# caslabuiowa/OptimalBezierTrajectoryGeneration

Measured on NVIDIA B200. Metric: constraint+Jacobian evals/sec, higher is better.
Workload: dtype f64

## Files before the change

### optimalbeziertrajectorygeneration_b200/csrc/common.cuh

```cuda
#pragma once
#include <cuda_runtime.h>
#include <stdint.h>
#include <stdio.h>
#include <string.h>

#include "bezgpu.h"

struct bez_plan {
    int n, dim, elev, device;
    int L;
    int Lh;
    int LhPad;
    double *d_PQ;
    double *d_T;
    double *d_W;
    double *d_E1;
    double h_W[(BEZ_MAX_DEGREE + 1) * (BEZ_MAX_DEGREE + 1)];
    double h_E1lo[BEZ_MAX_DEGREE + 1];
    double h_E1hi[BEZ_MAX_DEGREE + 1];
};

void bez_set_error(const char *fmt, ...);
int bez_cuda_fail(cudaError_t e, const char *what);

#define BEZ_CUDA(call)                                        \
    do {                                                      \
        cudaError_t e__ = (call);                             \
        if (e__ != cudaSuccess) return bez_cuda_fail(e__, #call); \
    } while (0)

struct BezDeviceGuard {
    int prev = -1;
    bool switched = false;
    cudaError_t err = cudaSuccess;
    explicit BezDeviceGuard(int device) {
        err = cudaGetDevice(&prev);
        if (err == cudaSuccess && prev != device) {
            err = cudaSetDevice(device);
            switched = (err == cudaSuccess);
        }
    }
    ~BezDeviceGuard() {
        if (switched) cudaSetDevice(prev);
    }
    BezDeviceGuard(const BezDeviceGuard &) = delete;
    BezDeviceGuard &operator=(const BezDeviceGuard &) = delete;
};
#define BEZ_ON_DEVICE(device)                                                     \
    BezDeviceGuard bez_guard__(device);                                            \
    if (bez_guard__.err != cudaSuccess) return bez_cuda_fail(bez_guard__.err, "cudaSetDevice")

int bez_kernel_config(const void *func, int threads, size_t shmem, int *sms, int *ctas_per_sm);

#define BEZ_REQUIRE(cond, msg)                 \
    do {                                       \
        if (!(cond)) {                         \
            bez_set_error("%s: %s", __func__, msg); \
            return BEZ_EINVAL;                 \
        }                                      \
    } while (0)

__host__ __device__ inline long long bez_pair_row_offset(long long i, long long N) {
    return i * (2 * N - i - 1) / 2;
}

__device__ inline void bez_pair_decode(long long p, int N, int &i, int &j) {
    const float b = 2.0f * (float)N - 1.0f;
    const float disc = (float)((2.0 * (double)N - 1.0) * (2.0 * (double)N - 1.0) - 8.0 * (double)p);
    int ii = (int)((b - __fsqrt_rn(disc > 0.0f ? disc : 0.0f)) * 0.5f);
    if (ii < 0) ii = 0;
    if (ii > N - 2) ii = N - 2;
    while (ii > 0 && bez_pair_row_offset(ii, N) > p) --ii;
    while (ii < N - 2 && bez_pair_row_offset(ii + 1, N) <= p) ++ii;
    i = ii;
    j = (int)(p - bez_pair_row_offset(ii, N)) + ii + 1;
}
```

### optimalbeziertrajectorygeneration_b200/csrc/plan.cu

```cuda
#include <stdarg.h>
#include <stdlib.h>

#include <mutex>
#include <vector>

#include "common.cuh"

static thread_local char g_err[512] = "";

void bez_set_error(const char *fmt, ...) {
    va_list ap;
    va_start(ap, fmt);
    vsnprintf(g_err, sizeof(g_err), fmt, ap);
    va_end(ap);
}

int bez_cuda_fail(cudaError_t e, const char *what) {
    bez_set_error("CUDA error %d (%s) in %s", (int)e, cudaGetErrorString(e), what);
    return (int)e;
}

extern "C" const char *bez_last_error(void) { return g_err; }

namespace {
struct KernelConfig {
    const void *func;
    int device, threads;
    size_t shmem;
    int sms, per_sm;
};
std::mutex g_cfg_mutex;
std::vector<KernelConfig> g_cfg;
}

int bez_kernel_config(const void *func, int threads, size_t shmem, int *sms, int *ctas_per_sm) {
    int dev = 0;
    BEZ_CUDA(cudaGetDevice(&dev));
    std::lock_guard<std::mutex> lock(g_cfg_mutex);
    for (const KernelConfig &c : g_cfg)
        if (c.func == func && c.device == dev && c.threads == threads && c.shmem == shmem) {
            *sms = c.sms;
            *ctas_per_sm = c.per_sm;
            return BEZ_OK;
        }
    KernelConfig c{func, dev, threads, shmem, 148, 1};
    size_t granted = 48 * 1024;
    for (const KernelConfig &o : g_cfg)
        if (o.func == func && o.device == dev && o.shmem > granted) granted = o.shmem;
    if (shmem > granted)
        BEZ_CUDA(cudaFuncSetAttribute(func, cudaFuncAttributeMaxDynamicSharedMemorySize, (int)shmem));
    BEZ_CUDA(cudaDeviceGetAttribute(&c.sms, cudaDevAttrMultiProcessorCount, dev));
    BEZ_CUDA(cudaOccupancyMaxActiveBlocksPerMultiprocessor(&c.per_sm, func, threads, shmem));
    if (c.per_sm < 1) c.per_sm = 1;
    g_cfg.push_back(c);
    *sms = c.sms;
    *ctas_per_sm = c.per_sm;
    return BEZ_OK;
}
extern "C" int bez_version(void) { return 100; }

extern "C" int bez_plan_create(int n, int dim, int elev, int device,
                               const double *h_prodW, const double *h_elevT,
                               const double *h_elev1, bez_plan **out) {
    BEZ_REQUIRE(out != nullptr, "out is NULL");
    *out = nullptr;
    BEZ_REQUIRE(h_prodW && h_elevT, "tables are NULL");
    BEZ_REQUIRE(dim >= 1 && dim <= 3, "dim must be 1, 2 or 3");
    BEZ_REQUIRE(elev >= 0, "elev must be >= 0");
    if (n < 1 || n > BEZ_MAX_DEGREE) {
        bez_set_error("bez_plan_create: degree %d outside [1, %d]", n, BEZ_MAX_DEGREE);
        return BEZ_EUNSUPPORTED;
    }
    BEZ_REQUIRE(h_elev1 != nullptr, "elev1 table is NULL");
    BEZ_ON_DEVICE(device);

    bez_plan *p = (bez_plan *)calloc(1, sizeof(bez_plan));
    if (!p) {
        bez_set_error("bez_plan_create: out of host memory");
        return BEZ_ENOMEM;
    }
    p->n = n; p->dim = dim; p->elev = elev; p->device = device;
    const int m = 2 * n;
    p->L = m + elev + 1;
    p->Lh = (p->L + 1) / 2;
    p->LhPad = (p->Lh + 31) / 32 * 32;
    const int L = p->L, M = m + elev;

    memcpy(p->h_W, h_prodW, sizeof(double) * (n + 1) * (n + 1));
    for (int i = 0; i <= n; ++i) {
        p->h_E1lo[i] = (i < n) ? h_elev1[i * (n + 1) + i] : 0.0;
        p->h_E1hi[i] = (i > 0) ? h_elev1[(i - 1) * (n + 1) + i] : 0.0;
    }

    std::vector<double> PQ((size_t)(m + 1) * p->LhPad, 0.0);
    for (int i = 0; i < p->Lh; ++i) {
        for (int j = 0; j < n; ++j) {
            double a = h_elevT[(size_t)j * L + i], b = h_elevT[(size_t)(m - j) * L + i];
            PQ[(size_t)j * p->LhPad + i] = (a + b) * 0.5;
            PQ[(size_t)(n + 1 + j) * p->LhPad + i] = (a - b) * 0.5;
        }
        PQ[(size_t)n * p->LhPad + i] = h_elevT[(size_t)n * L + i];
    }
    for (int i = p->Lh; i < p->LhPad; ++i) {
        const int mi = M - i;
        if (mi < 0 || mi >= p->Lh) continue;
        for (int j = 0; j <= n; ++j) PQ[(size_t)j * p->LhPad + i] = PQ[(size_t)j * p->LhPad + mi];
        for (int j = 0; j < n; ++j)
            PQ[(size_t)(n + 1 + j) * p->LhPad + i] = -PQ[(size_t)(n + 1 + j) * p->LhPad + mi];
    }

    cudaError_t e;
#define PLAN_ALLOC_COPY(dst, src, count)                                              \
    e = cudaMalloc((void **)&(dst), sizeof(double) * (count));                        \
    if (e == cudaSuccess)                                                             \
        e = cudaMemcpy((dst), (src), sizeof(double) * (count), cudaMemcpyHostToDevice); \
    if (e != cudaSuccess) { bez_plan_destroy(p); return bez_cuda_fail(e, "plan table upload"); }
    PLAN_ALLOC_COPY(p->d_PQ, PQ.data(), PQ.size());
    PLAN_ALLOC_COPY(p->d_T, h_elevT, (size_t)(m + 1) * L);
    PLAN_ALLOC_COPY(p->d_W, h_prodW, (size_t)(n + 1) * (n + 1));
    PLAN_ALLOC_COPY(p->d_E1, h_elev1, (size_t)n * (n + 1));
#undef PLAN_ALLOC_COPY
    *out = p;
    return BEZ_OK;
}

extern "C" int bez_plan_destroy(bez_plan *p) {
    if (!p) return BEZ_OK;
    cudaFree(p->d_PQ);
    cudaFree(p->d_T);
    cudaFree(p->d_W);
    cudaFree(p->d_E1);
    free(p);
    return BEZ_OK;
}

extern "C" int bez_plan_info(const bez_plan *p, int *n, int *dim, int *elev, int *L) {
    BEZ_REQUIRE(p != nullptr, "plan is NULL");
    if (n) *n = p->n;
    if (dim) *dim = p->dim;
    if (elev) *elev = p->elev;
    if (L) *L = p->L;
    return BEZ_OK;
}
```

### optimalbeziertrajectorygeneration_b200/csrc/sq_elev_ws.cuh

```cuda
#pragma once
#include "sq_elev_stage1.cuh"

namespace bezws {
using namespace bezcore;
using namespace bezmma;

constexpr int kProducers = 4, kConsumers = 8;
constexpr int kWsThreads = 32 * (kProducers + kConsumers);
constexpr int kSlots = 3;
constexpr int kBarsPerGroup = 3 * kSlots;

template <int R> __device__ __forceinline__ void reg_dec() { asm volatile("setmaxnreg.dec.sync.aligned.u32 %0;" :: "n"(R)); }
template <int R> __device__ __forceinline__ void reg_inc() { asm volatile("setmaxnreg.inc.sync.aligned.u32 %0;" :: "n"(R)); }
__device__ __forceinline__ void mbar_arrive(unsigned mbar_s) {
    asm volatile("mbarrier.arrive.shared::cta.b64 _, [%0];" :: "r"(mbar_s) : "memory");
}

template <int N_, int DIM> __host__ __device__ constexpr int slot_doubles() {
    constexpr int S_ = (DIM * (N_ + 1) + 1) / 2 * 2;
    return 32 * S_ > kRowsDoubles ? 32 * S_ : kRowsDoubles;
}

template <int N_, int DIM, int MINMODE, bool STORE>
__global__ void __launch_bounds__(kWsThreads, 1)
sq_elev_ws_kernel(const SqElevArgs A, const ProdWeights<N_> PW, const DiffWeights<N_> DW) {
    constexpr int NP = 4;
    constexpr int S_ = (DIM * (N_ + 1) + 1) / 2 * 2;
    constexpr int kSlotD = slot_doubles<N_, DIM>();
    extern __shared__ __align__(16) double smem[];
    const int lane = threadIdx.x & 31;
    const int warp = __shfl_sync(0xffffffffu, (int)(threadIdx.x >> 5), 0);
    const int group = warp & 3;
    double *slots = smem + (size_t)group * kSlots * kSlotD;
    double *stag0 = smem + (size_t)4 * kSlots * kSlotD;
    const size_t stag_per = STORE ? 16 * (size_t)A.L : 0;
    const unsigned bars_s = (unsigned)__cvta_generic_to_shared(stag0 + kConsumers * stag_per) + 8u * kBarsPerGroup * group;
    auto full_b = [&](int s) { return bars_s + 8u * s; };
    auto empty_b = [&](int s) { return bars_s + 8u * (kSlots + s); };
    auto rows_b = [&](int s) { return bars_s + 8u * (2 * kSlots + s); };
    if (warp < kProducers && lane == 0) {
        for (int s = 0; s < kSlots; ++s) { mbar_init(full_b(s), 32); mbar_init(empty_b(s), 32); mbar_init(rows_b(s), 1); }
        mbar_fence_init();
    }
    __syncthreads();

    const long long total = A.nitems * (long long)A.B;
    const long long nwt = (total + 31) >> 5;
    const long long ngroups = (long long)gridDim.x * 4, gidx = (long long)blockIdx.x * 4 + group;
    const long long t_begin = gidx * nwt / ngroups;
    const int n = (int)((gidx + 1) * nwt / ngroups - t_begin);

    if (warp < kProducers) {
        reg_dec<120>();
        PairCursor cur;
        if (n > 0) {
            const long long f = (t_begin << 5) + lane;
            cur = pair_cursor_at(A, f < total ? f : total - 1);
        }
        for (int k = 0; k < n; ++k) {
            const int s = k % kSlots, use = k / kSlots;
            double *slot = slots + (size_t)s * kSlotD;
            const unsigned slot_s = (unsigned)__cvta_generic_to_shared(slot);
            if (use > 0) mbar_wait(empty_b(s), (unsigned)(use - 1) & 1u);
            {
                const int pb = __shfl_up_sync(0xffffffffu, cur.b, 1), pi = __shfl_up_sync(0xffffffffu, cur.i, 1);
                const int pj = __shfl_up_sync(0xffffffffu, cur.j, 1);
                const bool start = lane == 0 || cur.b != pb || cur.i != pi || cur.j != pj + 1;
                const unsigned runs = __ballot_sync(0xffffffffu, start);
                if (lane == 0) mbar_arrive_expect_tx(rows_b(s), 32u * S_ * 8u);
                __syncwarp();
                if (start) {
                    const unsigned higher = lane == 31 ? 0u : (runs & (0xffffffffu << (lane + 1)));
                    const int end = higher ? __ffs(higher) - 1 : 32;
                    bulk_load(slot_s + (unsigned)lane * (S_ * 8u), A.cpts + ((size_t)cur.b * A.N + cur.j) * S_,
                              (unsigned)(end - lane) * (S_ * 8u), rows_b(s));
                }
            }
            const long long g0 = (t_begin + k) << 5;
            PairCursor nxt = cur;
            if (k + 1 < n) {
                const long long fn = g0 + 32 + lane;
                nxt = fn < total ? pair_cursor_next(A, cur, g0 + lane) : pair_cursor_at(A, total - 1);
            }
            mbar_wait(rows_b(s), (unsigned)use & 1u);
            double sc[2 * N_ + 1];
            stage1_coeffs<N_, DIM, PAIR, true>(A, PW, DW, cur.b, cur.i, cur.j, sc, slot + lane * S_);
            __syncwarp();
            double *row = slot + lane * kRowStride;
#pragma unroll
            for (int j = 0; j < N_; ++j) {
                row[slot_e(j)] = sc[j] + sc[2 * N_ - j];
                row[slot_o(j)] = sc[j] - sc[2 * N_ - j];
            }
            row[slot_e(N_)] = sc[N_];
#pragma unroll
            for (int j = N_ + 1; j < 4 * Geom<N_>::KE; ++j) row[slot_e(j)] = 0.0;
#pragma unroll
            for (int j = N_; j < 4 * Geom<N_>::KO; ++j) row[slot_o(j)] = 0.0;
            mbar_arrive(full_b(s));
            cur = nxt;
        }
    } else {
        reg_inc<192>();
        const int cidx = warp - kProducers, ci = cidx >> 2;
        double *obuf = stag0 + (size_t)cidx * stag_per;
        const unsigned obuf_s = (unsigned)__cvta_generic_to_shared(obuf);
        const bool base_aligned = (reinterpret_cast<uintptr_t>(A.out) & 15u) == 0;
        BFrags<N_, NP> Bf;
        load_bfrags<N_, NP>(Bf, A.PQ, A.L, A.LhPad, lane);
        for (int k = ci; k < n; k += 2) {
            const int s = k % kSlots, use = k / kSlots;
            const long long g0 = (t_begin + k) << 5;
            const int cnt = (int)((total - g0) < 32 ? (total - g0) : 32);
            mbar_wait(full_b(s), (unsigned)use & 1u);
            auto release = [&]() { mbar_arrive(empty_b(s)); };
            mma_tile<N_, NP, MINMODE, STORE, decltype(release)>(slots + (size_t)s * kSlotD, obuf, obuf_s, Bf,
                                                                STORE ? A.out + (size_t)g0 * A.L : nullptr, A.sinks, g0, cnt,
                                                                A.L, A.beta, lane, base_aligned, false, release);
            __syncwarp();
        }
        if (STORE && lane == 0) bulk_wait_all();
    }
}

template <int N_, int DIM> size_t ws_shmem_bytes(int L, bool store) {
    return ((size_t)4 * kSlots * slot_doubles<N_, DIM>() + (store ? (size_t)kConsumers * 16 * L : 0) + 4 * kBarsPerGroup) *
           sizeof(double);
}
template <int N_, int DIM> bool ws_fits(int L, bool store) { return ws_shmem_bytes<N_, DIM>(L, store) <= 232448; }

template <int N_, int DIM, int MINMODE, bool STORE>
int launch_sq_elev_ws(const bez_plan *plan, const SqElevArgs &A, cudaStream_t st) {
    ProdWeights<N_> PW;
    DiffWeights<N_> DW;
    const double scale = A.alpha * (0.5 * (double)DIM);
    for (int i = 0; i <= N_; ++i)
        for (int j = i; j <= N_; ++j) {
            double w = plan->h_W[i * (N_ + 1) + j] * scale;
            PW.w[widx<N_>(i, j)] = (i == j) ? w : 2.0 * w;
        }
    for (int i = 0; i <= N_; ++i) { DW.lo[i] = plan->h_E1lo[i]; DW.hi[i] = plan->h_E1hi[i]; }
    const size_t shmem = ws_shmem_bytes<N_, DIM>(A.L, STORE);
    auto kern = sq_elev_ws_kernel<N_, DIM, MINMODE, STORE>;
    int sms = 148, per_sm = 1;
    if (int rc = bez_kernel_config((const void *)kern, kWsThreads, shmem, &sms, &per_sm)) return rc;
    const long long nwt = (A.nitems * (long long)A.B + 31) / 32;
    long long grid = sms;
    if (grid > (nwt + 7) / 8) grid = (nwt + 7) / 8;
    if (grid == sms && grid > 1 && !(A.flags & kFlagFullGrid)) grid -= 1;
    if (grid < 1) return BEZ_OK;
    kern<<<(unsigned)grid, kWsThreads, shmem, st>>>(A, PW, DW);
    BEZ_CUDA(cudaGetLastError());
    return BEZ_OK;
}

}
```

Baseline: 12190.

## Replace static tile split in warp-specialized kernel with atomic dynamic work claiming

Each producer group now claims chunks of two 32-item tiles from a global atomic counter instead of taking a fixed contiguous range. Producers write the tile index into shared memory for consumers and send sentinel slots to end the loop. The last group to finish resets the counter, and each launch takes its counter pair from a ring on the plan. This is meant to even out load across groups when per-tile cost or group speed varies, at the cost of atomic traffic, a cursor re-seek at every chunk boundary, and a new launch-size limit.

```diff
diff --git a/optimalbeziertrajectorygeneration_b200/csrc/common.cuh b/optimalbeziertrajectorygeneration_b200/csrc/common.cuh
--- a/optimalbeziertrajectorygeneration_b200/csrc/common.cuh
+++ b/optimalbeziertrajectorygeneration_b200/csrc/common.cuh
@@ -18,7 +18,10 @@
     double h_W[(BEZ_MAX_DEGREE + 1) * (BEZ_MAX_DEGREE + 1)];
     double h_E1lo[BEZ_MAX_DEGREE + 1];
     double h_E1hi[BEZ_MAX_DEGREE + 1];
+    unsigned *d_ws_work;
+    mutable unsigned ws_work_next;
 };
+constexpr int kWsWorkRing = 64;
 
 void bez_set_error(const char *fmt, ...);
 int bez_cuda_fail(cudaError_t e, const char *what);
diff --git a/optimalbeziertrajectorygeneration_b200/csrc/plan.cu b/optimalbeziertrajectorygeneration_b200/csrc/plan.cu
--- a/optimalbeziertrajectorygeneration_b200/csrc/plan.cu
+++ b/optimalbeziertrajectorygeneration_b200/csrc/plan.cu
@@ -120,6 +120,10 @@
     PLAN_ALLOC_COPY(p->d_W, h_prodW, (size_t)(n + 1) * (n + 1));
     PLAN_ALLOC_COPY(p->d_E1, h_elev1, (size_t)n * (n + 1));
 #undef PLAN_ALLOC_COPY
+    e = cudaMalloc((void **)&p->d_ws_work, sizeof(unsigned) * 2 * kWsWorkRing);
+    if (e == cudaSuccess) e = cudaMemset(p->d_ws_work, 0, sizeof(unsigned) * 2 * kWsWorkRing);
+    if (e == cudaSuccess) e = cudaDeviceSynchronize();
+    if (e != cudaSuccess) { bez_plan_destroy(p); return bez_cuda_fail(e, "plan work counters"); }
     *out = p;
     return BEZ_OK;
 }
@@ -130,6 +134,7 @@
     cudaFree(p->d_T);
     cudaFree(p->d_W);
     cudaFree(p->d_E1);
+    cudaFree(p->d_ws_work);
     free(p);
     return BEZ_OK;
 }
diff --git a/optimalbeziertrajectorygeneration_b200/csrc/sq_elev_ws.cuh b/optimalbeziertrajectorygeneration_b200/csrc/sq_elev_ws.cuh
--- a/optimalbeziertrajectorygeneration_b200/csrc/sq_elev_ws.cuh
+++ b/optimalbeziertrajectorygeneration_b200/csrc/sq_elev_ws.cuh
@@ -9,6 +9,8 @@
 constexpr int kWsThreads = 32 * (kProducers + kConsumers);
 constexpr int kSlots = 3;
 constexpr int kBarsPerGroup = 3 * kSlots;
+constexpr int kWordsPerGroup = kBarsPerGroup + kSlots;
+constexpr int kChunk = 2;
 
 template <int R> __device__ __forceinline__ void reg_dec() { asm volatile("setmaxnreg.dec.sync.aligned.u32 %0;" :: "n"(R)); }
 template <int R> __device__ __forceinline__ void reg_inc() { asm volatile("setmaxnreg.inc.sync.aligned.u32 %0;" :: "n"(R)); }
@@ -23,7 +25,7 @@
 
 template <int N_, int DIM, int MINMODE, bool STORE>
 __global__ void __launch_bounds__(kWsThreads, 1)
-sq_elev_ws_kernel(const SqElevArgs A, const ProdWeights<N_> PW, const DiffWeights<N_> DW) {
+sq_elev_ws_kernel(const SqElevArgs A, const ProdWeights<N_> PW, const DiffWeights<N_> DW, unsigned *work) {
     constexpr int NP = 4;
     constexpr int S_ = (DIM * (N_ + 1) + 1) / 2 * 2;
     constexpr int kSlotD = slot_doubles<N_, DIM>();
@@ -34,30 +36,33 @@
     double *slots = smem + (size_t)group * kSlots * kSlotD;
     double *stag0 = smem + (size_t)4 * kSlots * kSlotD;
     const size_t stag_per = STORE ? 16 * (size_t)A.L : 0;
-    const unsigned bars_s = (unsigned)__cvta_generic_to_shared(stag0 + kConsumers * stag_per) + 8u * kBarsPerGroup * group;
+    long long *words = reinterpret_cast<long long *>(stag0 + kConsumers * stag_per) + kWordsPerGroup * group;
+    const unsigned bars_s = (unsigned)__cvta_generic_to_shared(words);
     auto full_b = [&](int s) { return bars_s + 8u * s; };
     auto empty_b = [&](int s) { return bars_s + 8u * (kSlots + s); };
     auto rows_b = [&](int s) { return bars_s + 8u * (2 * kSlots + s); };
+    int *tile_of = reinterpret_cast<int *>(words + 3 * kSlots);
+    const long long total = A.nitems * (long long)A.B;
+    const unsigned nwt = (unsigned)((total + 31) >> 5);
+    unsigned first = 0;
+    if (warp < kProducers && lane == 0) first = atomicAdd(work, (unsigned)kChunk);
     if (warp < kProducers && lane == 0) {
         for (int s = 0; s < kSlots; ++s) { mbar_init(full_b(s), 32); mbar_init(empty_b(s), 32); mbar_init(rows_b(s), 1); }
         mbar_fence_init();
     }
     __syncthreads();
 
-    const long long total = A.nitems * (long long)A.B;
-    const long long nwt = (total + 31) >> 5;
-    const long long ngroups = (long long)gridDim.x * 4, gidx = (long long)blockIdx.x * 4 + group;
-    const long long t_begin = gidx * nwt / ngroups;
-    const int n = (int)((gidx + 1) * nwt / ngroups - t_begin);
-
     if (warp < kProducers) {
         reg_dec<120>();
+        unsigned t = __shfl_sync(0xffffffffu, first, 0);
+        int pos = 0;
         PairCursor cur;
-        if (n > 0) {
-            const long long f = (t_begin << 5) + lane;
+        if (t < nwt) {
+            const long long f = ((long long)t << 5) + lane;
             cur = pair_cursor_at(A, f < total ? f : total - 1);
         }
-        for (int k = 0; k < n; ++k) {
+        int k = 0;
+        for (; t < nwt; ++k) {
             const int s = k % kSlots, use = k / kSlots;
             double *slot = slots + (size_t)s * kSlotD;
             const unsigned slot_s = (unsigned)__cvta_generic_to_shared(slot);
@@ -76,9 +81,12 @@
                               (unsigned)(end - lane) * (S_ * 8u), rows_b(s));
                 }
             }
-            const long long g0 = (t_begin + k) << 5;
+            const bool last = pos == kChunk - 1 || t + 1 == nwt;
+            unsigned claimed = 0;
+            if (last && lane == 0) claimed = atomicAdd(work, (unsigned)kChunk);
+            const long long g0 = (long long)t << 5;
             PairCursor nxt = cur;
-            if (k + 1 < n) {
+            if (!last) {
                 const long long fn = g0 + 32 + lane;
                 nxt = fn < total ? pair_cursor_next(A, cur, g0 + lane) : pair_cursor_at(A, total - 1);
             }
@@ -97,8 +105,34 @@
             for (int j = N_ + 1; j < 4 * Geom<N_>::KE; ++j) row[slot_e(j)] = 0.0;
 #pragma unroll
             for (int j = N_; j < 4 * Geom<N_>::KO; ++j) row[slot_o(j)] = 0.0;
+            if (lane == 0) tile_of[s] = (int)t;
             mbar_arrive(full_b(s));
+            if (last) {
+                t = __shfl_sync(0xffffffffu, claimed, 0);
+                pos = 0;
+                if (t < nwt) {
+                    const long long f = ((long long)t << 5) + lane;
+                    nxt = pair_cursor_at(A, f < total ? f : total - 1);
+                }
+            } else {
+                ++t;
+                ++pos;
+            }
             cur = nxt;
+        }
+        for (int e = 0; e < 2; ++e, ++k) {
+            const int s = k % kSlots, use = k / kSlots;
+            if (use > 0) mbar_wait(empty_b(s), (unsigned)(use - 1) & 1u);
+            if (lane == 0) tile_of[s] = -1;
+            mbar_arrive(full_b(s));
+        }
+        if (lane == 0) {
+            __threadfence();
+            if (atomicAdd(work + 1, 1u) == 4u * gridDim.x - 1) {
+                __threadfence();
+                atomicExch(work, 0u);
+                atomicExch(work + 1, 0u);
+            }
         }
     } else {
         reg_inc<192>();
@@ -108,11 +142,13 @@
         const bool base_aligned = (reinterpret_cast<uintptr_t>(A.out) & 15u) == 0;
         BFrags<N_, NP> Bf;
         load_bfrags<N_, NP>(Bf, A.PQ, A.L, A.LhPad, lane);
-        for (int k = ci; k < n; k += 2) {
+        for (int k = ci;; k += 2) {
             const int s = k % kSlots, use = k / kSlots;
-            const long long g0 = (t_begin + k) << 5;
+            mbar_wait(full_b(s), (unsigned)use & 1u);
+            const int t = tile_of[s];
+            if (t < 0) break;
+            const long long g0 = (long long)t << 5;
             const int cnt = (int)((total - g0) < 32 ? (total - g0) : 32);
-            mbar_wait(full_b(s), (unsigned)use & 1u);
             auto release = [&]() { mbar_arrive(empty_b(s)); };
             mma_tile<N_, NP, MINMODE, STORE, decltype(release)>(slots + (size_t)s * kSlotD, obuf, obuf_s, Bf,
                                                                 STORE ? A.out + (size_t)g0 * A.L : nullptr, A.sinks, g0, cnt,
@@ -124,7 +160,7 @@
 }
 
 template <int N_, int DIM> size_t ws_shmem_bytes(int L, bool store) {
-    return ((size_t)4 * kSlots * slot_doubles<N_, DIM>() + (store ? (size_t)kConsumers * 16 * L : 0) + 4 * kBarsPerGroup) *
+    return ((size_t)4 * kSlots * slot_doubles<N_, DIM>() + (store ? (size_t)kConsumers * 16 * L : 0) + 4 * kWordsPerGroup) *
            sizeof(double);
 }
 template <int N_, int DIM> bool ws_fits(int L, bool store) { return ws_shmem_bytes<N_, DIM>(L, store) <= 232448; }
@@ -149,7 +185,12 @@
     if (grid > (nwt + 7) / 8) grid = (nwt + 7) / 8;
     if (grid == sms && grid > 1 && !(A.flags & kFlagFullGrid)) grid -= 1;
     if (grid < 1) return BEZ_OK;
-    kern<<<(unsigned)grid, kWsThreads, shmem, st>>>(A, PW, DW);
+    if (nwt + 4 * grid * kChunk >= (1ll << 31)) {
+        bez_set_error("pair kernel: %lld items in one launch exceed the 2^36 limit", A.nitems * (long long)A.B);
+        return BEZ_EUNSUPPORTED;
+    }
+    const unsigned slot = __atomic_fetch_add(&plan->ws_work_next, 1u, __ATOMIC_RELAXED) % kWsWorkRing;
+    kern<<<(unsigned)grid, kWsThreads, shmem, st>>>(A, PW, DW, plan->d_ws_work + 2 * slot);
     BEZ_CUDA(cudaGetLastError());
     return BEZ_OK;
 }
```

Result: no change. 12110, median of 6 (-0.7%).
